# Exidekat/TransformerUpscaler

Hardware: AMD Instinct MI355X
Metric: images/sec, FastTransformer 2x 720p->1080p inference (higher is better)
Workload: dtype bf16

## Files before the change

include/tupscale_hip.h:

```cpp
#ifndef TUPSCALE_HIP_H
#define TUPSCALE_HIP_H

#ifdef __cplusplus
extern "C" {
#endif

int tup_abi_version(void);

int tup_conv3x3_c3_fwd(const float* x, const void* wp, const float* bias, const float* in_mask,
                       const void* out_mask, void* out, int B, int H, int W, int relu, void* stream);

int tup_conv3x3_c64_fwd(const void* x, const void* wp, const float* bias, const void* add,
                        const void* mask, void* out, int B, int H, int W, int ntiles, int r,
                        int cout_valid, int relu, int out_mode, int in_r, void* stream);

int tup_conv5x5_c64_planar_fwd(const void* x, const void* wp, const float* bias, const void* wv,
                               const float* bv, float* out, int B, int H, int W, int r, int relu, void* stream);

int tup_conv3x3_planar_fwd(const float* x, const float* w28, const float* bias, const float* add,
                           float* out, int B, int H, int W, int r, int clamp01, void* stream);

int tup_resize_aa_fwd(const float* in, float* out, const int* ymin, const int* ysize, const float* yw,
                      int KY, const int* xmin, const int* xsize, const float* xw, int KX, int planes,
                      int Hi, int Wi, int Ho, int Wo, int clamp01, void* stream);

int tup_tail_stream_r2_fwd(const float* x, const float* wfu_t, const float* bfu, const float* wfc_t, const float* bfc,
                           const float* ui, float* out, int B, int H, int W, int clamp01, void* stream);

int tup_tail_stream_r2_resize_fwd(const float* x, const float* wfu_t, const float* bfu, const float* wfc_t, const float* bfc,
                                  const float* ui, float* out, const int* ymin, const int* ysize, const float* yw, int KY,
                                  const int* xmin, const int* xsize, const float* xw, int KX, const int* oxb, const int* oyb,
                                  int B, int H, int W, int Ho, int Wo, int sc, int band_h, int ext, int clamp01, void* stream);

int tup_tail_fused_fwd(const float* x, const float* wfu, const float* bfu, const float* wfc, const float* bfc,
                       const float* ui, float* out, const int* ymin, const int* ysize, const float* yw, int KY,
                       const int* xmin, const int* xsize, const float* xw, int KX, int B, int H, int W, int r,
                       int Ho, int Wo, int EH, int EW, int clamp01, void* stream);

int tup_clamp01_fwd(const float* in, float* out, long long n, void* stream);

int tup_layernorm_fwd(const float* x, const float* gamma, const float* beta, void* y,
                      float* mean, float* rstd, int M, void* stream);

int tup_relpos_bias_expand(const float* table, float* frag, void* stream);

int tup_window_attn_fwd(const void* qkv, const float* bias_frag, void* out, float* lse, int nwin, float drop_p,
                        unsigned int drop_seed, void* stream);

int tup_gemm_tokens_fwd(const void* A, int a_dtype, int lda, const void* Wt, const float* bias,
                        const float* res, const void* aux, void* out, int ldo, int M, int N, int K,
                        int epilogue, float drop_p, unsigned int drop_seed, void* stream);

int tup_ln_gemm_fwd(const float* x, const float* gamma, const float* beta, const void* Wt,
                    const float* bias, void* out, int M, int N, void* stream);

int tup_fused_mlp_fwd(float* x, const float* gamma, const float* beta, const void* w1, const float* b1,
                      const void* w2, const float* b2, int M, void* stream);

int tup_patch_embed_fwd(const void* feat, const void* Wt, const float* bias, float* x_out,
                        int B, int H, int W, void* stream);

int tup_patch_unembed_fwd(const void* x, int x_bf16, const void* Wt, const float* bias, const void* skip,
                          void* out, int B, int H, int W, void* stream);


int tup_rt_patch_embed_fwd(const void* feat, const void* Wt, const float* bias, const float* pos, float* x_out,
                           int B, int H, int W, void* stream);
// ... 154 lines not shown
```

transformerupscaler_amd/_lib.py:

```python
from __future__ import annotations

import ctypes
import os
from ctypes import c_float, c_int, c_longlong, c_uint, c_void_p

_HERE = os.path.dirname(os.path.abspath(__file__))
LIB_PATH = os.environ.get("TUP_LIB_PATH") or os.path.join(_HERE, "libtupscale_hip.so")
ABI_VERSION = 15

P = c_void_p
I = c_int
F = c_float
U = c_uint

SIGNATURES = {
    "tup_abi_version": [],
    "tup_conv3x3_c3_fwd": [P, P, P, P, P, P, I, I, I, I, P],
    "tup_conv3x3_c64_fwd": [P, P, P, P, P, P, I, I, I, I, I, I, I, I, I, P],
    "tup_conv5x5_c64_planar_fwd": [P, P, P, P, P, P, I, I, I, I, I, P],
    "tup_conv3x3_planar_fwd": [P, P, P, P, P, I, I, I, I, I, P],
    "tup_resize_aa_fwd": [P, P, P, P, P, I, P, P, P, I, I, I, I, I, I, I, P],
    "tup_tail_fused_fwd": [P, P, P, P, P, P, P, P, P, P, I, P, P, P, I, I, I, I, I, I, I, I, I, I, P],
    "tup_tail_stream_r2_fwd": [P, P, P, P, P, P, P, I, I, I, I, P],
    "tup_tail_stream_r2_resize_fwd": [P] * 7 + [P, P, P, I, P, P, P, I, P, P] + [I] * 9 + [P],
    "tup_clamp01_fwd": [P, P, c_longlong, P],
    "tup_layernorm_fwd": [P, P, P, P, P, P, I, P],
    "tup_relpos_bias_expand": [P, P, P],
    "tup_window_attn_fwd": [P, P, P, P, I, F, U, P],
    "tup_gemm_tokens_fwd": [P, I, I, P, P, P, P, P, I, I, I, I, I, F, U, P],
    "tup_ln_gemm_fwd": [P, P, P, P, P, P, I, I, P],
    "tup_fused_mlp_fwd": [P, P, P, P, P, P, P, I, P],
    "tup_patch_embed_fwd": [P, P, P, P, I, I, I, P],
    "tup_patch_unembed_fwd": [P, I, P, P, P, P, I, I, I, P],
    "tup_rt_patch_embed_fwd": [P, P, P, P, P, I, I, I, P],
    "tup_rt_patch_unembed_fwd": [P, P, P, P, P, I, I, I, P],
    "tup_rt_attention_fwd": [P, P, P, I, I, F, U, P],
    "tup_rt_attention_bwd": [P, P, P, P, P, P, I, I, F, U, P],
    "tup_layernorm128_fwd": [P, P, P, P, P, P, I, P],
    "tup_layernorm128_bwd": [P, P, P, P, P, P, P, P, P, I, P, F, U, P],
    "tup_rt_patch_wgrad": [P, P, P, I, I, I, P],
    "tup_conv3x3_c64_wgrad_s2d": [P, P, P, P, I, I, I, I, I, P],
    "tup_rt_bicubic_bwd": [P] * 10 + [I, I, I, I, I, P],
    "tup_rt_bicubic_bwd_banded": [P] * 7 + [I, P, P, I, P, P, I, I, I, I, I, P, P],
    "tup_relpos_bias_expand_h": [P, P, I, P],
    "tup_relpos_bias_expand_n_h": [P, P, I, P],
    "tup_window_attn_bwd_h": [P, P, P, P, P, P, P, P, I, I, F, U, P],
    "tup_relpos_bias_reduce_h": [P, P, I, P],
    "tup_wt_patch_wgrad": [P, P, P, I, I, I, I, P],
    "tup_window_attn_fwd_h": [P, P, P, P, I, I, F, U, P],
    "tup_wt_patch_embed_fwd": [P, P, P, P, I, I, I, I, P],
    "tup_wt_patch_unembed_fwd": [P, P, P, P, P, I, I, I, I, P],
    "tup_fused_qkv_attn_fwd": [P, P, P, P, P, P, P, I, P],
    "tup_fused_attn_block_fwd": [P, P, P, P, P, P, P, P, I, P],
    "tup_fused_block_fwd": [P] * 10 + [I, P],
    "tup_fused_blocks32_fwd": [P, P, I, I, P],
    "tup_blocks_stream_fwd": [P, P, P, I, I, P],
    "tup_clock_probe": [P, P],
    "tup_pack_gather": [P, P, I, P, P, c_longlong, I, P],
    "tup_adam_step": [P, P, I, P],
    "tup_l1_loss_partial": [P, P, P, c_longlong, I, P],
    "tup_l1_loss_bwd": [P, P, P, P, c_longlong, P],
    "tup_u8hwc_to_f32chw": [P, P, I, I, I, I, P],
    "tup_f32chw_to_u8hwc": [P, P, I, I, I, I, P],
    "tup_bra_compose": [P, P, P, P, P, P, P, P],
    "tup_bra_backward": [P, P, P, P, P, P, P, P, P, I, I, I, P],
    "tup_bra_chain": [P, P, P, P, P, P, P, P, P, P, P],
    "tup_resize_u8_rows": [P, P, P, P, P, I, I, I, I, I, P],
    "tup_resize_u8_cols": [P, P, P, P, P, P, I, I, I, I, I, I, P],
    "tup_rt_bicubic_sum_fwd": [P, P, P, P, P, P, P, P, P, P, P, I, I, I, I, I, I, I, I, P],
    "tup_quality_f32_partial": [P, P, P, I, I, I, I, F, P],
    "tup_quality_u8hwc_partial": [P, P, P, I, I, I, I, F, P],
    "tup_quality_reduce": [P, P, I, I, I, I, F, P],
# ... 69 lines not shown
```

transformerupscaler_amd/csrc/check_resources.py:

```python
#!/usr/bin/env python3
import json
import os
import re
import subprocess
import sys

GUARDED = [
    ("fused_attn.hip", ["fused_qkv_attn_kernel"]),
    ("block_stream.hip", ["blocks_stream_kernel"]),
    ("fused_blocks.hip", ["fused_mlp_v2_kernel"]),
    ("conv3x3_c64.hip", ["conv_c64_persistent_kernel", "bra_rows_persistent_kernel", "conv3_thin_rows_kernel"]),
    ("conv_thin.hip", ["conv3x3_c3_persistent_kernel"]),
    ("gemm_tokens.hip", ["gemm_panel2_kernel", "patch_embed_kernel"]),
    ("conv_bwd.hip", ["conv3x3_wgrad_c64_kernel", "conv3x3_wgrad_thin_kernel"]),
    ("branch_a_train.hip", ["bra_wgrad_kernel"]),
    ("gemm_wgrad.hip", ["gemm_wgrad_wide_kernel"]),
]
EXEMPT = re.compile(r"fused_qkv_attn_kernel<true, true, true>|fused_qkv_attn_kernelILb1ELb1ELb1E|fused_mlp_v2_kernelILi[1-9]|blocks_stream_kernel<true>|blocks_stream_kernelILb1E")
ALLOWED_BYTES = {"fused_mlp_v2_kernelILi0E": 72}

FIELDS = {
    "sgprs": r"TotalSGPRs: (\d+)", "vgprs": r" VGPRs: (\d+)", "agprs": r"AGPRs: (\d+)",
    "scratch_bytes_per_lane": r"ScratchSize \[bytes/lane\]: (\d+)", "waves_per_simd": r"Occupancy \[waves/SIMD\]: (\d+)",
    "sgpr_spill": r"SGPRs Spill: (\d+)", "vgpr_spill": r"VGPRs Spill: (\d+)",
}


def demangle(names):
    try:
        out = subprocess.run(["c++filt"], input="\n".join(names), capture_output=True, text=True, check=True).stdout.split("\n")
        return dict(zip(names, out))
    except Exception:
        return {n: n for n in names}


def parse(path):
    txt = open(path, errors="replace").read()
    parts = re.split(r"remark: Function Name: (\S+)", txt)
    recs = {}
    for name, body in zip(parts[1::2], parts[2::2]):
        rec = {}
        for k, pat in FIELDS.items():
            m = re.search(pat, body)
            if m:
                rec[k] = int(m.group(1))
        recs[name] = rec
    return recs


def main(argv):
    out_path = None
    files = []
    for a in argv:
        if a.startswith("--out="):
            out_path = a[6:]
        else:
            files.append(a)
    report, bad = {}, []
    for f in sorted(files):
        src = os.path.basename(f).replace(".remarks", ".hip")
        recs = parse(f)
        names = demangle(list(recs))
        for mangled, rec in recs.items():
            nice = names.get(mangled, mangled)
            rec["source"] = src
# ... 32 lines not shown
```

transformerupscaler_amd/engine.py:

```python
from __future__ import annotations

import os

import math
from typing import Dict, Optional, Tuple

import torch

from . import ops
from .weights import BLOCKS, VALID_SCALES, upsampler_layout


stage_timer = None
fuse_attention = 3


class _NullCtx:
    def __enter__(self):
        return None

    def __exit__(self, *a):
        return False


def _stage(name: str):
    return stage_timer(name) if stage_timer is not None else _NullCtx()


def resolve_scale(h: int, w: int, res_out, upscale_factor: Optional[int]):
    if upscale_factor is not None:
        res_out = (h * upscale_factor, w * upscale_factor)
    else:
        upscale_factor = math.ceil(max(res_out[0] / h, res_out[1] / w))
    if upscale_factor not in VALID_SCALES:
        raise ValueError(f"Requested scale={upscale_factor} was not built.")
    return (int(res_out[0]), int(res_out[1])), int(upscale_factor)


blocks_in_one_launch = True
stream_blocks = True
STREAM_MIN_WINDOWS = 512
stream_bf16_tokens = True
fuse_blocks = True
fuse_tail = True
stream_tail = True


def _block_operands(pk, i, bias_frags):
    return (pk[f"b{i}.qkv.whn"], pk[f"b{i}.qkv.bhn"], bias_frags[i], pk[f"b{i}.proj.wpp"], pk[f"b{i}.proj.b"],
            pk[f"b{i}.fc1.wfqn"], pk[f"b{i}.fc1.bqn"], pk[f"b{i}.fc2.wh4"], pk[f"b{i}.fc2.b"])


def transformer_blocks(pk: Dict[str, torch.Tensor], x: torch.Tensor, bias_frags, capture=None, bf16_out: bool = False):
    if (fuse_blocks and fuse_attention >= 3 and capture is None and "b0.stream.0" in pk and blocks_in_one_launch and stream_blocks
            and x.shape[0] // 64 >= STREAM_MIN_WINDOWS):
        table = ops.stream_table([tuple(pk[f"b{i}.stream.{j}"] for j in range(7)) for i in range(BLOCKS)])
        return ops.blocks_stream(x, table, out_bf16=bf16_out and stream_bf16_tokens)
    if fuse_blocks and fuse_attention >= 3 and capture is None and "b0.proj.wpp" in pk and blocks_in_one_launch:
        table = ops.block_table([_block_operands(pk, i, bias_frags) for i in range(BLOCKS)])
        return ops.fused_blocks32(x, table)
    for i in range(BLOCKS):
        qkv = None
        if fuse_blocks and fuse_attention >= 3 and capture is None and f"b{i}.proj.wpp" in pk:
            ops.fused_block(x, *_block_operands(pk, i, bias_frags))
            continue
        if fuse_blocks and fuse_attention == 2 and capture is None and f"b{i}.proj.wpp" in pk:
            ops.fused_attn_block(x, pk[f"b{i}.norm1.w"], pk[f"b{i}.norm1.b"], pk[f"b{i}.qkv.wh"], pk[f"b{i}.qkv.bh"], bias_frags[i],
                                 pk[f"b{i}.proj.wpp"], pk[f"b{i}.proj.b"])
            ops.fused_mlp(x, pk[f"b{i}.norm2.w"], pk[f"b{i}.norm2.b"], pk[f"b{i}.fc1.wfq"], pk[f"b{i}.fc1.bq"],
                          pk[f"b{i}.fc2.wh4"], pk[f"b{i}.fc2.b"])
            continue
        if fuse_blocks and fuse_attention and capture is None and f"b{i}.qkv.wh" in pk:
            att = ops.fused_qkv_attn(x, pk[f"b{i}.norm1.w"], pk[f"b{i}.norm1.b"], pk[f"b{i}.qkv.wh"], pk[f"b{i}.qkv.bh"], bias_frags[i])
        else:
            if fuse_blocks:
                qkv = ops.ln_gemm(x, pk[f"b{i}.norm1.w"], pk[f"b{i}.norm1.b"], pk[f"b{i}.qkv.w"], pk[f"b{i}.qkv.b"])
            else:
                y = ops.layernorm(x, pk[f"b{i}.norm1.w"], pk[f"b{i}.norm1.b"])
                qkv = ops.gemm_tokens(y, pk[f"b{i}.qkv.w"], pk[f"b{i}.qkv.b"], "bf16")
            att = ops.window_attn(qkv, bias_frags[i])
        ops.gemm_tokens(att, pk[f"b{i}.proj.w"], pk[f"b{i}.proj.b"], "res", res=x, out=x)
        if fuse_blocks and f"b{i}.fc1.wfq" in pk:
            ops.fused_mlp(x, pk[f"b{i}.norm2.w"], pk[f"b{i}.norm2.b"], pk[f"b{i}.fc1.wfq"], pk[f"b{i}.fc1.bq"],
                          pk[f"b{i}.fc2.wh4"], pk[f"b{i}.fc2.b"])
        else:
            y = ops.layernorm(x, pk[f"b{i}.norm2.w"], pk[f"b{i}.norm2.b"])
            hid = ops.gemm_tokens(y, pk[f"b{i}.fc1.w"], pk[f"b{i}.fc1.b"], "gelu")
            ops.gemm_tokens(hid, pk[f"b{i}.fc2.w"], pk[f"b{i}.fc2.b"], "res", res=x, out=x)
        if capture is not None:
            capture[f"block{i}"] = x.clone()
            capture[f"block{i}_qkv"] = qkv
            capture[f"block{i}_attn_out"] = att
    return x


def forward(pk: Dict[str, torch.Tensor], bias_frags, x: torch.Tensor, scale: int, res_out: Tuple[int, int],
            require_ratio: bool = True, capture: Optional[dict] = None, fuse_branch_a: bool = True) -> torch.Tensor:
    cap = capture
    x = x.contiguous().float()
    B, _, H, W = x.shape
    with _stage("conv1"):
        feat1 = ops.conv1(x, pk["conv1.w"], pk["conv1.b"], relu=True)
    with _stage("conv2"):
        feat = ops.conv_c64(feat1, pk["conv2.w"], pk["conv2.b"], 1, relu=True)
    del feat1
    stages = upsampler_layout(scale)
    up = feat
    if fuse_branch_a and "bra.w" in pk:
        for si, (_, r) in enumerate(stages[:-1]):
            up = ops.conv_c64(up, pk[f"up1.{si}.w"], pk[f"up1.{si}.b"], r, relu=False)
        with _stage("branch_a"):
            upscaled_input = ops.branch_a_composed(up, pk["bra.w"], pk["bra.b"], pk["bra.wv"], pk["bra.bv"], stages[-1][1])
    else:
        for si, (_, r) in enumerate(stages):
            with _stage(f"up1.{si}"):
                up = ops.conv_c64(up, pk[f"up1.{si}.w"], pk[f"up1.{si}.b"], r, relu=False)
        upscaled_input = ops.conv_c64_thin(up, pk["up1_conv.w"], None, 3, relu=True)
        if cap is not None:
            cap["up1"] = up
    if cap is not None:
        cap["feat"] = feat; cap["upscaled_input"] = upscaled_input
    del up
    with _stage("patch_embed"):
        xw = ops.patch_embed(feat, pk["pe.w"], pk["pe.b"])
    if cap is not None:
        cap["win_in"] = xw.clone()
    with _stage("blocks"):
        xw = transformer_blocks(pk, xw, bias_frags, cap, bf16_out=cap is None)
    with _stage("unembed"):
        combined = ops.patch_unembed(xw, pk["pu.w"], pk["pu.b"], feat)
    with _stage("dec1"):
        dec = ops.conv_c64(combined, pk["dec1.w"], pk["dec1.b"], 1, relu=True)
    with _stage("dec2"):
        residual = ops.conv_c64_thin(dec, pk["dec2.w"], pk["dec2.b"], 3, relu=False)
    if cap is not None:
        cap["combined"] = combined; cap["dec"] = dec; cap["residual"] = residual
    t = residual
    hs, ws = H * scale, W * scale
    needs_resize = bool(require_ratio) and tuple(res_out) != (hs, hs) and tuple(res_out) != (hs, ws)
    fu = upsampler_layout(scale)
    if fuse_tail and cap is None:
        for si, (_, r) in enumerate(fu[:-1]):
            t = ops.conv_planar(t, pk[f"fu.{si}.w"], pk[f"fu.{si}.b"], r)
        li = len(fu) - 1
        if (stream_tail and fu[li][1] == 2 and "tail.wfu_t" in pk
                and ops.tail_stream_fits(t.shape[0], t.shape[2], t.shape[3], tuple(res_out) if needs_resize else None)):
            with _stage("tail"):
                out = ops.tail_stream_r2(t, pk["tail.wfu_t"], pk[f"fu.{li}.b"], pk["tail.wfc_t"], pk["fuc.b"], upscaled_input,
                                         clamp=True, out_hw=tuple(res_out) if needs_resize else None)
                if out is None:
                    out = ops.tail_stream_r2(t, pk["tail.wfu_t"], pk[f"fu.{li}.b"], pk["tail.wfc_t"], pk["fuc.b"], upscaled_input, clamp=False)
                    out = ops.resize_aa(out, tuple(res_out), clamp=True)
            return out
        with _stage("tail"):
            out = ops.tail_fused(t, pk[f"fu.{li}.w"], pk[f"fu.{li}.b"], pk["fuc.w"], pk["fuc.b"], upscaled_input, fu[li][1],
                                 tuple(res_out) if needs_resize else (hs, ws), clamp=True)
        return out
    for si, (_, r) in enumerate(fu):
        t = ops.conv_planar(t, pk[f"fu.{si}.w"], pk[f"fu.{si}.b"], r)
    out = ops.conv_planar(t, pk["fuc.w"], pk["fuc.b"], 1, add=upscaled_input, clamp=not needs_resize)
    if cap is not None:
        cap["sum"] = out
    if needs_resize:
        out = ops.resize_aa(out, res_out, clamp=True)
    return out
```

transformerupscaler_amd/ops.py:

```python
from __future__ import annotations

import os

import numpy as np
import torch

from . import _lib
from .resize_taps import aa_taps

BF16, F32 = torch.bfloat16, torch.float32


_raw_stream = getattr(torch._C, "_cuda_getCurrentRawStream", None)
_cur_dev = torch.cuda.current_device


def _stream():
    if _raw_stream is not None:
        return _raw_stream(_cur_dev())
    return torch.cuda.current_stream().cuda_stream


def _chk(t: torch.Tensor, dtype, shape=None, name="tensor"):
    if t.dtype != dtype:
# ... 25 lines not shown


def zero_pool_end():
    global _zero_pool
    _zero_pool = None


def _zeros(shape, device):
    n = 1
    for d in shape:
        n *= int(d)
    zp = _zero_pool
    if zp is not None and zp[0].device == torch.device(device) and zp[1] + n <= zp[0].numel():
        off = zp[1]
        zp[1] = off + ((n + 63) // 64) * 64
        return zp[0][off:off + n].view(shape)
    return torch.zeros(shape, dtype=F32, device=device)


def conv1(x, wp, bias, relu=True, in_mask=None, out_mask=None):
    B, C, H, W = x.shape
    assert C == 3
    out = torch.empty((B, H, W, 64), dtype=BF16, device=x.device)
    _lib.call("tup_conv3x3_c3_fwd", _chk(x, F32, None, "x"), _chk(wp, BF16, (64, 32), "wp"),
              _opt(bias, F32, (64,), "bias"), _opt(in_mask, F32, x.shape, "in_mask"),
              _opt(out_mask, BF16, out.shape, "out_mask"), out.data_ptr(), B, H, W, int(relu), _stream())
    return out


def conv_c64(x, wp, bias, r=1, relu=False, add=None, mask=None, in_r=1, out=None):
    B, Hi, Wi, C = x.shape
    assert C == 64 and Hi % in_r == 0 and Wi % in_r == 0
    H, W = Hi // in_r, Wi // in_r
    nt = r * r
    if out is None:
        out = torch.empty((B, H * r, W * r, 64), dtype=BF16, device=x.device)
    else:
        _chk(out, BF16, (B, H * r, W * r, 64), "out")
    _lib.call("tup_conv3x3_c64_fwd", _chk(x, BF16, None, "x"), _chk(wp, BF16, (nt, in_r * in_r, 9, 64, 64), "wp"),
              _opt(bias, F32, (nt, 64), "bias"), _opt(add, BF16, out.shape, "add"), _opt(mask, BF16, out.shape, "mask"),
              out.data_ptr(), B, H, W, nt, r, 64, int(relu), 0, in_r, _stream())
    return out


def conv_c64_thin(x, wp, bias, cout, relu=False, out=None):
    B, H, W, C = x.shape
    assert C == 64 and 1 <= cout <= 16
    if out is None:
        out = torch.empty((B, cout, H, W), dtype=F32, device=x.device)
    else:
        _chk(out, F32, (B, cout, H, W), "out")
    _lib.call("tup_conv3x3_c64_fwd", _chk(x, BF16, None, "x"), _chk(wp, BF16, (1, 1, 9, 16, 64), "wp"),
              _opt(bias, F32, (cout,), "bias"), None, None, out.data_ptr(), B, H, W, 1, 1, cout, int(relu), 1, 1, _stream())
    return out


def branch_a_composed(x, wp, bias, wv, bv, r, relu=True):
    B, H, W, C = x.shape
    assert C == 64 and r in (2, 3, 6)
    rows, n = {2: 16, 3: 32, 6: 112}[r], 3 * r * r
    out = torch.empty((B, 3, H * r, W * r), dtype=F32, device=x.device)
    _lib.call("tup_conv5x5_c64_planar_fwd", _chk(x, BF16, None, "x"), _chk(wp, BF16, (1, 1, 25, rows, 64), "wp"),
              _chk(bias, F32, (n,), "bias"), _chk(wv, BF16, (9, n, 25, 64), "wv"), _chk(bv, F32, (9, n), "bv"),
              out.data_ptr(), B, H, W, r, int(relu), _stream())
    return out


def conv_planar(x, w28, bias, r=1, add=None, clamp=False):
    B, C, H, W = x.shape
    assert C == 3
    cout = 3 * r * r
    both = clamp == "both"
    shape = (B, 3, H * r, W * r)
    out = torch.empty(((2,) if both else ()) + shape, dtype=F32, device=x.device)
    _lib.call("tup_conv3x3_planar_fwd", _chk(x, F32, None, "x"), _chk(w28, F32, (cout, 28), "w28"),
              _opt(bias, F32, (cout,), "bias"), _opt(add, F32, shape, "add"), out.data_ptr(),
              B, H, W, r, 2 if both else int(bool(clamp)), _stream())
    return (out[0], out[1]) if both else out


_TAP_CACHE = {}


def _taps_on(device, in_size, out_size):
    key = (str(device), in_size, out_size)
    if key not in _TAP_CACHE:
        lo, n, w, k = aa_taps(in_size, out_size)
        _TAP_CACHE[key] = (torch.from_numpy(lo).to(device), torch.from_numpy(n).to(device),
                           torch.from_numpy(w).to(device), k)
    return _TAP_CACHE[key]


def resize_aa(x, size, clamp=False):
    B, C, Hi, Wi = x.shape
    Ho, Wo = size
    ylo, yn, yw, ky = _taps_on(x.device, Hi, Ho)
    xlo, xn, xw, kx = _taps_on(x.device, Wi, Wo)
    both = clamp == "both"
    out = torch.empty(((2,) if both else ()) + (B, C, Ho, Wo), dtype=F32, device=x.device)
    _lib.call("tup_resize_aa_fwd", _chk(x, F32, None, "x"), out.data_ptr(), ylo.data_ptr(), yn.data_ptr(),
              yw.data_ptr(), ky, xlo.data_ptr(), xn.data_ptr(), xw.data_ptr(), kx, B * C, Hi, Wi, Ho, Wo,
              2 if both else int(bool(clamp)), _stream())
    return (out[0], out[1]) if both else out


TAIL_TILE_H = 16
# ... 900 lines not shown
```

transformerupscaler_amd/packing.py:

```python
from __future__ import annotations

from typing import Dict

import torch

from .weights import BLOCKS, upsampler_layout

_PERM64 = torch.tensor([((n >> 2) & 3) * 16 + (n >> 4) * 4 + (n & 3) for n in range(64)], dtype=torch.long)


_IDX_CACHE: Dict[tuple, torch.Tensor] = {}


def _dev_index(key, build, device) -> torch.Tensor:
    k = (key, str(device))
    t = _IDX_CACHE.get(k)
    if t is None:
        t = _IDX_CACHE[k] = build().to(device)
    return t


def _perm64(device) -> torch.Tensor:
    return _dev_index("perm64", lambda: _PERM64, device)


def perm_rows64(w: torch.Tensor) -> torch.Tensor:
    n = w.shape[0]
    assert n % 64 == 0
    idx = _dev_index(("rows64", n), lambda: (torch.arange(n // 64).view(-1, 1) * 64 + _PERM64.view(1, -1)).reshape(-1), w.device)
    return w.index_select(0, idx)


def pack_conv_c64(weight: torch.Tensor, bias, r: int):
    cout, cin = weight.shape[0], weight.shape[1]
    assert cin == 64 and cout == 64 * r * r and weight.shape[2:] == (3, 3)
    w = weight.reshape(64, r * r, 64, 9)
    w = w.permute(1, 3, 0, 2)
    w = w.index_select(2, _perm64(w.device))
    b = None if bias is None else bias.reshape(64, r * r).t().contiguous().float()
    return w.unsqueeze(1).contiguous().to(torch.bfloat16), b


def pack_conv_c64_thin(weight: torch.Tensor):
    co = weight.shape[0]
    assert weight.shape[1] == 64 and co <= 16
    w = torch.zeros(9, 16, 64, dtype=weight.dtype, device=weight.device)
    w[:, :co, :] = weight.reshape(co, 64, 9).permute(2, 0, 1)
    return w.view(1, 1, 9, 16, 64).contiguous().to(torch.bfloat16)


def pack_conv1(weight: torch.Tensor):
    assert tuple(weight.shape) == (64, 3, 3, 3)
    w = torch.zeros(64, 32, dtype=weight.dtype, device=weight.device)
    w[:, :27] = weight.permute(0, 2, 3, 1).reshape(64, 27)
    return perm_rows64(w).contiguous().to(torch.bfloat16)


def pack_planar(weight: torch.Tensor):
    cout = weight.shape[0]
    assert weight.shape[1:] == (3, 3, 3)
    w = torch.zeros(cout, 28, dtype=torch.float32, device=weight.device)
    w[:, :27] = weight.reshape(cout, 27).float()
    return w.contiguous()


def pack_planar_t(weight: torch.Tensor):
    cout = weight.shape[0]
    assert weight.shape[1:] == (3, 3, 3)
    w = torch.zeros(27, (cout + 3) // 4 * 4, dtype=torch.float32, device=weight.device)
    w[:, :cout] = weight.reshape(cout, 27).float().t()
    return w.contiguous()


def pack_linear(weight: torch.Tensor):
    return perm_rows64(weight).contiguous().to(torch.bfloat16)


def pack_linear_stack(weights, transpose: bool = False):
    w = torch.stack([t.detach() for t in weights])
    if transpose:
        w = w.transpose(1, 2)
    n = w.shape[1]
    assert n % 64 == 0
    idx = _dev_index(("rows64", n), lambda: (torch.arange(n // 64).view(-1, 1) * 64 + _PERM64.view(1, -1)).reshape(-1), w.device)
    return w.index_select(1, idx).to(torch.bfloat16)


def pack_fc1_fused(weight: torch.Tensor):
    return pack_linear(weight).index_select(1, _fused_k_order(weight.device)).contiguous()


def pack_fc1_fused_q(weight: torch.Tensor, bias: torch.Tensor):
    return pack_fc1_fused(weight.detach() * 0.25), (bias.detach().float() * 0.25).contiguous()


def pack_fc2_h4(weight: torch.Tensor):
    return perm_rows64(weight.detach() * 4.0).contiguous().to(torch.float16)


def fold_layernorm(weight: torch.Tensor, bias: torch.Tensor, gamma: torch.Tensor, beta: torch.Tensor):
    w = weight.detach().float()
# ... 199 lines not shown
        k = f"up1.upsamplers.{scale}.{idx}"
        pk[f"up1.{si}.w"], pk[f"up1.{si}.b"] = pack_conv_c64(sd[k + ".weight"].detach(), sd[k + ".bias"].detach(), r)
        k = f"final_upscale.upsamplers.{scale}.{idx}"
        pk[f"fu.{si}.w"] = pack_planar(sd[k + ".weight"].detach()); pk[f"fu.{si}.b"] = f32(sd[k + ".bias"])
    pk["up1_conv.w"] = pack_conv_c64_thin(sd["up1_conv.conv.weight"].detach())
    if not backward:
        idx, r = upsampler_layout(scale)[-1]
        k = f"up1.upsamplers.{scale}.{idx}"
        pk["bra.w"], pk["bra.b"], pk["bra.wv"], pk["bra.bv"] = pack_branch_a(
            sd[k + ".weight"].detach(), sd[k + ".bias"].detach(), sd["up1_conv.conv.weight"].detach(), r)
    pk["fuc.w"] = pack_planar(sd["final_upscale_conv.weight"].detach()); pk["fuc.b"] = f32(sd["final_upscale_conv.bias"])
    if not backward and upsampler_layout(scale)[-1][1] == 2:
        li = len(upsampler_layout(scale)) - 1
        pk["tail.wfu_t"] = pack_planar_t(sd[f"final_upscale.upsamplers.{scale}.{upsampler_layout(scale)[-1][0]}.weight"].detach())
        pk["tail.wfc_t"] = pack_planar_t(sd["final_upscale_conv.weight"].detach())
    pk["pe.w"] = pack_patch_embed(sd["patch_embed.weight"].detach()); pk["pe.b"] = f32(sd["patch_embed.bias"])
    for i in range(BLOCKS):
        p = f"window_blocks.{i}"
        for nm in ("norm1", "norm2"):
            pk[f"b{i}.{nm}.w"] = f32(sd[f"{p}.{nm}.weight"]); pk[f"b{i}.{nm}.b"] = f32(sd[f"{p}.{nm}.bias"])
        pk[f"b{i}.table"] = f32(sd[f"{p}.attn.relative_position_bias_table"])
        for nm, key in (("qkv", "attn.qkv"), ("proj", "attn.proj"), ("fc1", "mlp.0"), ("fc2", "mlp.2")):
            pk[f"b{i}.{nm}.b"] = f32(sd[f"{p}.{key}.bias"])
    for nm, key in (("qkv", "attn.qkv"), ("proj", "attn.proj"), ("fc1", "mlp.0"), ("fc2", "mlp.2")):
        ws = [sd[f"window_blocks.{i}.{key}.weight"] for i in range(BLOCKS)]
        wp = pack_linear_stack(ws)
        for i in range(BLOCKS):
            pk[f"b{i}.{nm}.w"] = wp[i]
        if backward:
            wt = pack_linear_stack(ws, transpose=True)
            for i in range(BLOCKS):
                pk[f"b{i}.{nm}.wd"] = wt[i]
    if not backward:
        for i in range(BLOCKS):
            p = f"window_blocks.{i}"
            pk[f"b{i}.qkv.wh"], pk[f"b{i}.qkv.bh"] = pack_qkv_heads(sd[f"{p}.attn.qkv.weight"], sd[f"{p}.attn.qkv.bias"])
            pk[f"b{i}.proj.wpp"] = pack_proj_pairs(sd[f"{p}.attn.proj.weight"])
            pk[f"b{i}.fc1.wfq"], pk[f"b{i}.fc1.bq"] = pack_fc1_fused_q(sd[f"{p}.mlp.0.weight"], sd[f"{p}.mlp.0.bias"])
            pk[f"b{i}.qkv.whn"], pk[f"b{i}.qkv.bhn"] = pack_qkv_heads(*fold_layernorm(
                sd[f"{p}.attn.qkv.weight"], sd[f"{p}.attn.qkv.bias"], sd[f"{p}.norm1.weight"], sd[f"{p}.norm1.bias"]))
            pk[f"b{i}.fc1.wfqn"], pk[f"b{i}.fc1.bqn"] = pack_fc1_fused_q(*fold_layernorm(
                sd[f"{p}.mlp.0.weight"], sd[f"{p}.mlp.0.bias"], sd[f"{p}.norm2.weight"], sd[f"{p}.norm2.bias"]))
            pk[f"b{i}.fc2.wh4"] = pack_fc2_h4(sd[f"window_blocks.{i}.mlp.2.weight"])
            for j, t in enumerate(pack_stream_block(
                    sd[f"{p}.attn.qkv.weight"], sd[f"{p}.attn.qkv.bias"], sd[f"{p}.norm1.weight"], sd[f"{p}.norm1.bias"],
                    sd[f"{p}.attn.relative_position_bias_table"], sd[f"{p}.attn.proj.weight"], sd[f"{p}.attn.proj.bias"],
                    sd[f"{p}.mlp.0.weight"], sd[f"{p}.mlp.0.bias"], sd[f"{p}.norm2.weight"], sd[f"{p}.norm2.bias"],
                    sd[f"{p}.mlp.2.weight"], sd[f"{p}.mlp.2.bias"])):
                pk[f"b{i}.stream.{j}"] = t
    pk["pu.w"] = pack_patch_unembed(sd["patch_unembed.weight"].detach()); pk["pu.b"] = f32(sd["patch_unembed.bias"])
    pk["dec1.w"], pk["dec1.b"] = pack_conv_c64(sd["decoder_conv1.weight"].detach(), sd["decoder_conv1.bias"].detach(), 1)
    pk["dec2.w"] = pack_conv_c64_thin(sd["decoder_conv2.weight"].detach()); pk["dec2.b"] = f32(sd["decoder_conv2.bias"])
    if not backward:
        return pk
    t = lambda k: sd[k].detach()
    pk["conv1.wd"] = pack_conv_c64_thin(t("conv1.weight").flip(2, 3).transpose(0, 1).contiguous())
    pk["conv2.wd"] = pack_conv_c64_dgrad(t("conv2.weight"), 1)
    pk["dec1.wd"] = pack_conv_c64_dgrad(t("decoder_conv1.weight"), 1)
    pk["dec2.wd"] = pack_conv_thin_dgrad(t("decoder_conv2.weight"))
    pk["up1_conv.wd"] = pack_conv_thin_dgrad(t("up1_conv.conv.weight"))
    pk["fuc.wd"] = pack_planar_dgrad(t("final_upscale_conv.weight"))
    for si, (idx, r) in enumerate(upsampler_layout(scale)):
        pk[f"up1.{si}.wd"] = pack_conv_c64_dgrad(t(f"up1.upsamplers.{scale}.{idx}.weight"), r)
        pk[f"fu.{si}.raw"] = f32(sd[f"final_upscale.upsamplers.{scale}.{idx}.weight"])
    pk["pe.wd"] = pack_linear(t("patch_embed.weight").permute(2, 3, 1, 0).reshape(4096, 192))
    pk["pu.wd"] = pack_linear(t("patch_unembed.weight").permute(0, 2, 3, 1).reshape(192, 4096))
    return pk


def pack_conv_c64_stride2(weight: torch.Tensor, bias):
    assert tuple(weight.shape) == (64, 64, 3, 3)
    w = torch.zeros(4, 9, 64, 64, dtype=weight.dtype, device=weight.device)
    for si in range(2):
        for sj in range(2):
            for dy in range(3):
                for dx in range(3):
                    ky, kx = 2 * (dy - 1) + si + 1, 2 * (dx - 1) + sj + 1
                    if 0 <= ky <= 2 and 0 <= kx <= 2:
                        w[si * 2 + sj, dy * 3 + dx] = weight[:, :, ky, kx]
    w = w.index_select(2, _perm64(w.device))
    b = None if bias is None else bias.reshape(1, 64).contiguous().float()
    return w.unsqueeze(0).contiguous().to(torch.bfloat16), b


def pack_conv_c64_stride2_dgrad(weight: torch.Tensor):
    assert tuple(weight.shape) == (64, 64, 3, 3)
    w = torch.zeros(4, 9, 64, 64, dtype=weight.dtype, device=weight.device)
    for si in range(2):
        for sj in range(2):
            for dy in range(3):
                for dx in range(3):
                    ky, kx = si + 1 - 2 * (dy - 1), sj + 1 - 2 * (dx - 1)
                    if 0 <= ky <= 2 and 0 <= kx <= 2:
                        w[si * 2 + sj, dy * 3 + dx] = weight[:, :, ky, kx].t()
    w = w.index_select(2, _perm64(w.device))
    return w.unsqueeze(1).contiguous().to(torch.bfloat16)


def unpack_conv_c64_stride2_wgrad(dwp: torch.Tensor):
    dw = torch.zeros(64, 64, 3, 3, dtype=dwp.dtype, device=dwp.device)
    for si in range(2):
        for sj in range(2):
            for dy in range(3):
                for dx in range(3):
                    ky, kx = 2 * (dy - 1) + si + 1, 2 * (dx - 1) + sj + 1
                    if 0 <= ky <= 2 and 0 <= kx <= 2:
# ... 78 lines not shown
```

Measured before the change: 2353.

## Fuse decoder conv1 and conv2 into one persistent kernel with seam fixup

```diff
diff --git a/include/tupscale_hip.h b/include/tupscale_hip.h
--- a/include/tupscale_hip.h
+++ b/include/tupscale_hip.h
@@ -13,6 +13,9 @@
 int tup_conv3x3_c64_fwd(const void* x, const void* wp, const float* bias, const void* add,
                         const void* mask, void* out, int B, int H, int W, int ntiles, int r,
                         int cout_valid, int relu, int out_mode, int in_r, void* stream);
+
+int tup_decoder_fused_fwd(const void* x, const void* w1, const float* b1, const void* wz, const float* b2,
+                          float* seamv, float* cseam, float* out, int B, int H, int W, void* stream);
 
 int tup_conv5x5_c64_planar_fwd(const void* x, const void* wp, const float* bias, const void* wv,
                                const float* bv, float* out, int B, int H, int W, int r, int relu, void* stream);
diff --git a/transformerupscaler_amd/_lib.py b/transformerupscaler_amd/_lib.py
--- a/transformerupscaler_amd/_lib.py
+++ b/transformerupscaler_amd/_lib.py
@@ -18,6 +18,7 @@
     "tup_conv3x3_c3_fwd": [P, P, P, P, P, P, I, I, I, I, P],
     "tup_conv3x3_c64_fwd": [P, P, P, P, P, P, I, I, I, I, I, I, I, I, I, P],
     "tup_conv5x5_c64_planar_fwd": [P, P, P, P, P, P, I, I, I, I, I, P],
+    "tup_decoder_fused_fwd": [P, P, P, P, P, P, P, P, I, I, I, P],
     "tup_conv3x3_planar_fwd": [P, P, P, P, P, I, I, I, I, I, P],
     "tup_resize_aa_fwd": [P, P, P, P, P, I, P, P, P, I, I, I, I, I, I, I, P],
     "tup_tail_fused_fwd": [P, P, P, P, P, P, P, P, P, P, I, P, P, P, I, I, I, I, I, I, I, I, I, I, P],
diff --git a/transformerupscaler_amd/csrc/check_resources.py b/transformerupscaler_amd/csrc/check_resources.py
--- a/transformerupscaler_amd/csrc/check_resources.py
+++ b/transformerupscaler_amd/csrc/check_resources.py
@@ -11,6 +11,7 @@
     ("fused_blocks.hip", ["fused_mlp_v2_kernel"]),
     ("conv3x3_c64.hip", ["conv_c64_persistent_kernel", "bra_rows_persistent_kernel", "conv3_thin_rows_kernel"]),
     ("conv_thin.hip", ["conv3x3_c3_persistent_kernel"]),
+    ("decoder_fused.hip", ["decoder_fused_kernel"]),
     ("gemm_tokens.hip", ["gemm_panel2_kernel", "patch_embed_kernel"]),
     ("conv_bwd.hip", ["conv3x3_wgrad_c64_kernel", "conv3x3_wgrad_thin_kernel"]),
     ("branch_a_train.hip", ["bra_wgrad_kernel"]),
diff --git a/transformerupscaler_amd/csrc/decoder_fused.hip b/transformerupscaler_amd/csrc/decoder_fused.hip
--- /dev/null
+++ b/transformerupscaler_amd/csrc/decoder_fused.hip
@@ -0,0 +1,343 @@
+#include "common.h"
+
+namespace {
+
+constexpr int TH = 8, TW = 32, HALO_W = TW + 2, HALO_H = TH + 2, NPIX_HALO = HALO_H * HALO_W;
+constexpr int IN_BYTES = NPIX_HALO * 128, IN_CHUNKS = NPIX_HALO * 8;
+constexpr int WROWS = 64, WSLAB = WROWS * 128, WCHUNKS = 9 * WROWS * 8;
+constexpr size_t DEC_LDS = (size_t)9 * WSLAB + 2 * (size_t)IN_BYTES + 256;
+static_assert(DEC_LDS <= 163840, "LDS budget");
+
+__device__ __attribute__((aligned(16))) unsigned int dec_zero_line[4] = {0u, 0u, 0u, 0u};
+
+#define TUP_ADD_DPP(a, v, ctrl) asm("v_add_f32_dpp %0, %1, %0 " ctrl " row_mask:0xf bank_mask:0xf bound_ctrl:1" : "+v"(a) : "v"(v))
+
+__global__ __launch_bounds__(512, 2) void decoder_fused_kernel(
+    const bf16_t* __restrict__ x, const bf16_t* __restrict__ wp, const float* __restrict__ bias,
+    const bf16_t* __restrict__ wz, float* __restrict__ part, float* __restrict__ seamv, float* __restrict__ cseam,
+    int B, int H, int W, int tilesX, int tilesY)
+{
+    extern __shared__ __attribute__((aligned(16))) char smem[];
+    char* w_lds = smem;
+    char* in_lds = smem + 9 * WSLAB;
+
+    const int grp = __builtin_amdgcn_readfirstlane((int)(threadIdx.x >> 8));
+    const int tid = threadIdx.x & 255, lane = tid & 63, wave = tid >> 6;
+    const int g = lane >> 4, p = lane & 15;
+    const int total_tiles = tilesX * tilesY * B;
+    char* my_in = in_lds + grp * IN_BYTES;
+
+    constexpr int NPIECE = (IN_CHUNKS + 255) / 256;
+    int rel[NPIECE];
+#pragma unroll
+    for (int it = 0; it < NPIECE; ++it) {
+        const int idx = min(it * 256 + tid, IN_CHUNKS - 1);
+        const int q = idx >> 3, c = (idx & 7) ^ ((q >> 1) & 7);
+        const int yy = q / HALO_W, xx = q - yy * HALO_W;
+        rel[it] = ((yy - 1) * W + (xx - 1)) * 128 + c * 16;
+    }
+    const bool last_ok = (NPIECE - 1) * 256 + tid < IN_CHUNKS;
+    struct TC { int tx, ty, b; };
+    auto prefetch_tile = [&](const TC& c) {
+        const int ty0 = c.ty * TH, tx0 = c.tx * TW;
+        const char* xb = reinterpret_cast<const char*>(x + (size_t)c.b * H * W * 64);
+        if (ty0 >= 1 && ty0 + TH + 1 <= H && tx0 >= 1 && tx0 + TW + 1 <= W) {
+            const char* tb = xb + ((size_t)ty0 * W + tx0) * 128;
+#pragma unroll
+            for (int it = 0; it < NPIECE; ++it) {
+                if (it == NPIECE - 1 && !last_ok) continue;
+                __builtin_amdgcn_global_load_lds((const __attribute__((address_space(1))) void*)(tb + rel[it]),
+                                                 (__attribute__((address_space(3))) void*)(my_in + (it * 256 + wave * 64) * 16), 16, 0, 0);
+            }
+            return;
+        }
+#pragma unroll 1
+        for (int base = 0; base < IN_CHUNKS; base += 256) {
+            const int idx = base + tid;
+            if (idx < IN_CHUNKS) {
+                const int q = idx >> 3, cphys = idx & 7;
+                const int c = cphys ^ ((q >> 1) & 7);
+                const int yy = q / HALO_W, xx = q - yy * HALO_W;
+                const int iy = ty0 - 1 + yy, ix = tx0 - 1 + xx;
+                const void* src = (iy >= 0 && iy < H && ix >= 0 && ix < W)
+                                      ? (const void*)(xb + ((size_t)(iy * W + ix) * 128 + c * 16)) : (const void*)dec_zero_line;
+                __builtin_amdgcn_global_load_lds((const __attribute__((address_space(1))) void*)src,
+                                                 (__attribute__((address_space(3))) void*)(my_in + (base + wave * 64) * 16), 16, 0, 0);
+            }
+        }
+    };
+
+    uint32_t poff[9][2];
+#pragma unroll
+    for (int tap = 0; tap < 9; ++tap)
+#pragma unroll
+        for (int rw = 0; rw < 2; ++rw)
+            poff[tap][rw] = lds_addr(my_in) + (uint32_t)swz128((2 * wave + rw) * HALO_W + p + (tap / 3) * HALO_W + (tap % 3), g);
+    const uint32_t wbase0 = lds_addr(w_lds) + (uint32_t)swz128(p, g), wbase1 = wbase0 ^ 64u;
+    const uint32_t wbase0h = wbase0 + 57344u, wbase1h = wbase1 + 57344u;
+
+    f32x4 acc[4][4];
+    float* bias_lds = reinterpret_cast<float*>(in_lds + 2 * IN_BYTES);
+    const uint32_t bias_addr = lds_addr(bias_lds) + (uint32_t)(g * 64);
+    bf16x8 zf[3][2];
+    const uint32_t wz_voff = (uint32_t)(p * 128 + g * 16);
+    auto load_zf = [&]() {
+#pragma unroll
+        for (int dy = 0; dy < 3; ++dy) {
+            const bf16_t* base = wz + dy * 1024;
+            asm volatile("global_load_dwordx4 %0, %1, %2" : "=v"(zf[dy][0]) : "v"(wz_voff), "s"(base));
+            asm volatile("global_load_dwordx4 %0, %1, %2 offset:64" : "=v"(zf[dy][1]) : "v"(wz_voff), "s"(base));
+        }
+    };
+
+    auto compute_tile = [&]() {
+#pragma unroll
+        for (int ct = 0; ct < 4; ++ct) acc[0][ct] = __builtin_bit_cast(f32x4, lds_read_b128_asm(bias_addr + ct * 16));
+        lds_wait<0>();
+#pragma unroll
+        for (int pg = 1; pg < 4; ++pg)
+#pragma unroll
+            for (int ct = 0; ct < 4; ++ct) acc[pg][ct] = acc[0][ct];
+        constexpr int NSTEPS = 18, PER = 8;
+        bf16x8 pf[3][4], wf[3][4];
+        auto load_one = [&](int step, int slot, int j) {
+            const int tap = step >> 1;
+            if (j < 4) {
+                pf[slot][j] = (step & 1) ? lds_read_b128_asm_off_x64(poff[tap][j >> 1], (j & 1) * 2048)
+                                         : lds_read_b128_asm_off(poff[tap][j >> 1], (j & 1) * 2048);
+            } else {
+                const int woff = (tap * WROWS + (j - 4) * 16) * 128;
+                wf[slot][j - 4] = woff < 57344 ? lds_read_b128_asm_off((step & 1) ? wbase1 : wbase0, woff)
+                                               : lds_read_b128_asm_off((step & 1) ? wbase1h : wbase0h, woff - 57344);
+            }
+        };
+#pragma unroll
+        for (int j = 0; j < PER; ++j) load_one(0, 0, j);
+#pragma unroll
+        for (int j = 0; j < PER; ++j) load_one(1, 1, j);
+#pragma unroll
+        for (int step = 0; step < NSTEPS; ++step) {
+            const int cur = step % 3;
+            if (step + 1 < NSTEPS) lds_wait<PER>(); else lds_wait<0>();
+            __builtin_amdgcn_sched_barrier(0);
+            int rd = 0;
+#pragma unroll
+            for (int m = 0; m < 16; ++m) {
+                if (step + 2 < NSTEPS) {
+#pragma unroll
+                    for (int j = 0; j < PER; ++j)
+                        if (j == rd && j * 16 <= m * PER) { load_one(step + 2, (step + 2) % 3, j); ++rd; }
+                }
+                const int pg = m / 4, ct = m % 4;
+                acc[pg][ct] = mfma16x16x32(wf[cur][ct], pf[cur][pg], acc[pg][ct]);
+                __builtin_amdgcn_sched_barrier(0);
+            }
+        }
+    };
+
+    auto store_tile = [&](const TC& c) {
+        const int b = c.b, y0 = c.ty * TH + 2 * wave, x0 = c.tx * TW;
+        const bool edge = c.ty * TH + TH > H || x0 + TW > W;
+        f32x4 z[4][3];
+#pragma unroll
+        for (int pg = 0; pg < 4; ++pg) {
+            typedef short s16x2 __attribute__((ext_vector_type(2)));
+            uint32_t pk[8];
+#pragma unroll
+            for (int ct = 0; ct < 4; ++ct) {
+                pk[ct * 2 + 0] = pack_bf16x2(acc[pg][ct][0], acc[pg][ct][1]);
+                pk[ct * 2 + 1] = pack_bf16x2(acc[pg][ct][2], acc[pg][ct][3]);
+            }
+#pragma unroll
+            for (int q = 0; q < 8; ++q)
+                pk[q] = __builtin_bit_cast(uint32_t, __builtin_elementwise_max(__builtin_bit_cast(s16x2, pk[q]), s16x2{0, 0}));
+            if (edge) {
+                const bool ok = y0 + (pg >> 1) < H && x0 + (pg & 1) * 16 + p < W;
+#pragma unroll
+                for (int q = 0; q < 8; ++q) pk[q] = ok ? pk[q] : 0u;
+            }
+            const bf16x8 b0 = __builtin_bit_cast(bf16x8, u32x4{pk[0], pk[1], pk[2], pk[3]});
+            const bf16x8 b1 = __builtin_bit_cast(bf16x8, u32x4{pk[4], pk[5], pk[6], pk[7]});
+#pragma unroll
+            for (int dy = 0; dy < 3; ++dy) {
+                z[pg][dy] = mfma16x16x32(zf[dy][0], b0, f32x4{0.f, 0.f, 0.f, 0.f});
+                z[pg][dy] = mfma16x16x32(zf[dy][1], b1, z[pg][dy]);
+            }
+        }
+        __builtin_amdgcn_sched_barrier(0);
+        asm volatile("s_nop 7\n\ts_nop 7\n\ts_nop 4" ::: "memory");
+        __builtin_amdgcn_sched_barrier(0);
+        float h[2][2][3];
+#pragma unroll
+        for (int rw = 0; rw < 2; ++rw)
+#pragma unroll
+            for (int dy = 0; dy < 3; ++dy) {
+                const f32x4 l = z[2 * rw][dy], r = z[2 * rw + 1][dy];
+                float v0 = l[1], v1 = r[1];
+                TUP_ADD_DPP(v0, l[0], "row_shr:1"); TUP_ADD_DPP(v0, l[2], "row_shl:1"); TUP_ADD_DPP(v0, r[2], "row_shr:15");
+                TUP_ADD_DPP(v1, r[0], "row_shr:1"); TUP_ADD_DPP(v1, r[2], "row_shl:1"); TUP_ADD_DPP(v1, l[0], "row_shl:15");
+                h[rw][0][dy] = v0; h[rw][1][dy] = v1;
+            }
+        const bool live = g < 3;
+        const int plane = H * W, nrec = 3 * plane * 4;
+        const __amdgpu_buffer_rsrc_t rp = __builtin_amdgcn_make_buffer_rsrc(part + (size_t)b * 3 * plane, 0, nrec, 0x00020000);
+        const __amdgpu_buffer_rsrc_t rs = __builtin_amdgcn_make_buffer_rsrc(seamv + (size_t)b * 3 * plane, 0, nrec, 0x00020000);
+        const int crec = H * tilesX * 128;
+        const __amdgpu_buffer_rsrc_t rc = __builtin_amdgcn_make_buffer_rsrc(cseam + (size_t)b * H * tilesX * 32, 0, crec, 0x00020000);
+        const int cbase = (g * plane + y0 * W) * 4;
+#pragma unroll
+        for (int cg = 0; cg < 2; ++cg) {
+            const int ox = x0 + cg * 16 + p;
+            const bool colok = live && ox < W;
+            const int o = cbase + ox * 4, rowb = W * 4;
+            const float o0 = h[0][cg][1] + h[1][cg][2], o1 = h[0][cg][0] + h[1][cg][1];
+            __builtin_amdgcn_raw_buffer_store_b32(__builtin_bit_cast(uint32_t, o0), rp, colok && y0 < H ? o : nrec, 0, 0);
+            __builtin_amdgcn_raw_buffer_store_b32(__builtin_bit_cast(uint32_t, o1), rp, colok && y0 + 1 < H ? o + rowb : nrec, 0, 0);
+            __builtin_amdgcn_raw_buffer_store_b32(__builtin_bit_cast(uint32_t, h[0][cg][2]), rs,
+                                                  colok && y0 >= 1 && y0 < H ? o - rowb : nrec, 0, 0);
+            __builtin_amdgcn_raw_buffer_store_b32(__builtin_bit_cast(uint32_t, h[1][cg][0]), rs,
+                                                  colok && y0 + 2 < H ? o + 2 * rowb : nrec, 0, 0);
+        }
+#pragma unroll
+        for (int rw = 0; rw < 2; ++rw) {
+            const int y = y0 + rw;
+            const bool left = p == 0;
+            const f32x4 v = left ? f32x4{z[2 * rw][0][2], z[2 * rw][1][2], z[2 * rw][2][2], 0.f}
+                                 : f32x4{z[2 * rw + 1][0][0], z[2 * rw + 1][1][0], z[2 * rw + 1][2][0], 0.f};
+            const bool ok = live & (y < H) & (left | ((p == 15) & (x0 + TW <= W)));
+            const int off = ((y * tilesX + c.tx) * 2 + (left ? 0 : 1)) * 64 + g * 16;
+            __builtin_amdgcn_raw_buffer_store_b128(__builtin_bit_cast(u32x4, v), rc, ok ? off : crec, 0, 0);
+        }
+    };
+    constexpr int NSTORES = 10;
+
+    int first, first0, stride, limit;
+    if ((gridDim.x & 7) == 0) {
+        const int per = gridDim.x >> 3, band = (total_tiles + 7) >> 3, start = (blockIdx.x & 7) * band;
+        limit = min(total_tiles, start + band);
+        first0 = start + (blockIdx.x >> 3);
+        first = first0 + grp * per;
+        stride = 2 * per;
+    } else {
+        limit = total_tiles;
+        first0 = blockIdx.x;
+        first = first0 + grp * gridDim.x;
+        stride = 2 * gridDim.x;
+    }
+    const int my_count = first < limit ? (limit - first + stride - 1) / stride : 0;
+    const int cnt0 = first0 < limit ? (limit - first0 + stride - 1) / stride : 0;
+    const int nphases = 2 * cnt0 + 1;
+    TC c_first;
+    { const int t = first / tilesX; c_first.tx = first - t * tilesX; c_first.ty = t % tilesY; c_first.b = t / tilesY; }
+    const int step_x = stride % tilesX, step_y = (stride / tilesX) % tilesY, step_b = stride / (tilesX * tilesY);
+    auto advance = [&](TC& c) {
+        c.tx += step_x;
+        if (c.tx >= tilesX) { c.tx -= tilesX; ++c.ty; }
+        c.ty += step_y; c.b += step_b;
+        if (c.ty >= tilesY) { c.ty -= tilesY; ++c.b; }
+    };
+
+    for (int idx = threadIdx.x; idx < WCHUNKS; idx += 512) {
+        const int row = idx >> 3, c = idx & 7;
+        *reinterpret_cast<u32x4*>(w_lds + swz128(row, c)) = *reinterpret_cast<const u32x4*>(wp + (size_t)idx * 8);
+    }
+    if (threadIdx.x < 64) {
+        const int gg = threadIdx.x >> 4, ct = (threadIdx.x >> 2) & 3, e = threadIdx.x & 3;
+        bias_lds[threadIdx.x] = bias[gg * 16 + ct * 4 + e];
+    }
+    if (grp == 0 && my_count > 0) prefetch_tile(c_first);
+    __syncthreads();
+    TC c_done = c_first, c_next = c_first;
+    if (grp == 0) advance(c_next);
+
+    for (int ph = 0; ph < nphases; ++ph) {
+        const int k = ph >> 1;
+        if ((ph & 1) == grp) {
+            if (k < my_count) compute_tile();
+        } else {
+            const int done = grp == 0 ? k : k - 1;
+            const int nxt = done + 1;
+            const bool store = done >= 0 && done < my_count;
+            const bool fetch = nxt < my_count;
+            if (store) load_zf();
+            if (fetch) prefetch_tile(c_next);
+            if (store) {
+                if (fetch) asm volatile("s_waitcnt vmcnt(%0)" ::"n"(NPIECE - 1) : "memory");
+                else asm volatile("s_waitcnt vmcnt(0)" ::: "memory");
+                store_tile(c_done);
+                asm volatile("s_waitcnt vmcnt(%0)" ::"n"(NSTORES) : "memory");
+            } else {
+                asm volatile("s_waitcnt vmcnt(0)" ::: "memory");
+            }
+            c_done = c_next;
+            advance(c_next);
+        }
+        asm volatile("s_waitcnt lgkmcnt(0)" ::: "memory");
+        __builtin_amdgcn_s_barrier();
+    }
+    asm volatile("s_waitcnt vmcnt(0)" ::: "memory");
+}
+
+template <int V>
+__global__ __launch_bounds__(256) void decoder_finish_kernel(
+    float* __restrict__ res, const float* __restrict__ seamv, const float* __restrict__ cseam, const float* __restrict__ bias,
+    int H, int W, int tilesX)
+{
+    typedef float fv __attribute__((ext_vector_type(V)));
+    const int x0 = (blockIdx.x * 256 + threadIdx.x) * V;
+    if (x0 >= W) return;
+    const int row = blockIdx.y, b = row / H, y = row - b * H;
+    const size_t plane = (size_t)H * W;
+    const int ys = (y & 1) ? y + 1 : y - 1;
+    const bool has_seam = ys >= 0 && ys < H;
+    const size_t o0 = (size_t)b * 3 * plane + (size_t)y * W + x0;
+#pragma unroll
+    for (int c = 0; c < 3; ++c) {
+        const size_t o = o0 + c * plane;
+        fv v = *reinterpret_cast<const fv*>(res + o);
+        const fv sv = has_seam ? *reinterpret_cast<const fv*>(seamv + o) : fv{};
+#pragma unroll
+        for (int e = 0; e < V; ++e) {
+            const int xq = x0 + e;
+            float t = bias[c] + v[e];
+            if (has_seam) t += sv[e];
+            int ctile = -1, side = 0;
+            if ((xq & 31) == 31 && xq + 1 < W) { ctile = (xq >> 5) + 1; side = 0; }
+            else if ((xq & 31) == 0 && xq > 0) { ctile = (xq >> 5) - 1; side = 1; }
+            if (ctile >= 0) {
+#pragma unroll
+                for (int dy = 0; dy < 3; ++dy) {
+                    const int yy = y + dy - 1;
+                    if (yy >= 0 && yy < H) t += cseam[((((size_t)b * H + yy) * tilesX + ctile) * 2 + side) * 16 + c * 4 + dy];
+                }
+            }
+            v[e] = t;
+        }
+        *reinterpret_cast<fv*>(res + o) = v;
+    }
+}
+
+}
+
+extern "C" int tup_decoder_fused_fwd(const void* x, const void* w1, const float* b1, const void* wz, const float* b2,
+                                     float* seamv, float* cseam, float* out, int B, int H, int W, void* stream)
+{
+    if (B <= 0 || H <= 0 || W <= 0) return 0;
+    const int tilesX = (W + TW - 1) / TW, tilesY = (H + TH - 1) / TH;
+    const long long nt = (long long)tilesX * tilesY * B;
+    if (nt > 0x7fffffffLL || (long long)H * W * 12 > 0x7fffffffLL || (long long)H * tilesX * 128 > 0x7fffffffLL)
+        return (int)hipErrorInvalidValue;
+    hipStream_t s = reinterpret_cast<hipStream_t>(stream);
+    TUP_SET_DYN_LDS(decoder_fused_kernel, DEC_LDS);
+    const int grid = (int)(nt < 256 ? nt : 256);
+    decoder_fused_kernel<<<dim3(grid), dim3(512), DEC_LDS, s>>>((const bf16_t*)x, (const bf16_t*)w1, b1, (const bf16_t*)wz, out,
+                                                                 seamv, cseam, B, H, W, tilesX, tilesY);
+    TUP_CHECK_LAUNCH();
+    if ((long long)B * H > 0x7fffffffLL) return (int)hipErrorInvalidValue;
+    if (W % 4 == 0)
+        decoder_finish_kernel<4><<<dim3((unsigned)((W / 4 + 255) / 256), (unsigned)(B * H)), dim3(256), 0, s>>>(out, seamv, cseam, b2, H, W, tilesX);
+    else
+        decoder_finish_kernel<1><<<dim3((unsigned)((W + 255) / 256), (unsigned)(B * H)), dim3(256), 0, s>>>(out, seamv, cseam, b2, H, W, tilesX);
+    TUP_CHECK_LAUNCH();
+    return 0;
+}
diff --git a/transformerupscaler_amd/engine.py b/transformerupscaler_amd/engine.py
--- a/transformerupscaler_amd/engine.py
+++ b/transformerupscaler_amd/engine.py
@@ -44,6 +44,7 @@
 fuse_blocks = True
 fuse_tail = True
 stream_tail = True
+fuse_decoder = True
 
 
 def _block_operands(pk, i, bias_frags):
@@ -129,10 +130,14 @@
         xw = transformer_blocks(pk, xw, bias_frags, cap, bf16_out=cap is None)
     with _stage("unembed"):
         combined = ops.patch_unembed(xw, pk["pu.w"], pk["pu.b"], feat)
-    with _stage("dec1"):
-        dec = ops.conv_c64(combined, pk["dec1.w"], pk["dec1.b"], 1, relu=True)
-    with _stage("dec2"):
-        residual = ops.conv_c64_thin(dec, pk["dec2.w"], pk["dec2.b"], 3, relu=False)
+    if fuse_decoder and fuse_tail and cap is None and "dec2.wz" in pk:
+        with _stage("decoder"):
+            residual = ops.decoder_fused(combined, pk["dec1.w"], pk["dec1.b"], pk["dec2.wz"], pk["dec2.b"])
+    else:
+        with _stage("dec1"):
+            dec = ops.conv_c64(combined, pk["dec1.w"], pk["dec1.b"], 1, relu=True)
+        with _stage("dec2"):
+            residual = ops.conv_c64_thin(dec, pk["dec2.w"], pk["dec2.b"], 3, relu=False)
     if cap is not None:
         cap["combined"] = combined; cap["dec"] = dec; cap["residual"] = residual
     t = residual
diff --git a/transformerupscaler_amd/ops.py b/transformerupscaler_amd/ops.py
--- a/transformerupscaler_amd/ops.py
+++ b/transformerupscaler_amd/ops.py
@@ -101,6 +101,18 @@
         _chk(out, F32, (B, cout, H, W), "out")
     _lib.call("tup_conv3x3_c64_fwd", _chk(x, BF16, None, "x"), _chk(wp, BF16, (1, 1, 9, 16, 64), "wp"),
               _opt(bias, F32, (cout,), "bias"), None, None, out.data_ptr(), B, H, W, 1, 1, cout, int(relu), 1, 1, _stream())
+    return out
+
+
+def decoder_fused(x, w1, b1, wz, b2):
+    B, H, W, C = x.shape
+    assert C == 64
+    out = torch.empty((B, 3, H, W), dtype=F32, device=x.device)
+    seamv = torch.empty((B, 3, H, W), dtype=F32, device=x.device)
+    cseam = torch.empty((B, H, (W + 31) // 32, 32), dtype=F32, device=x.device)
+    _lib.call("tup_decoder_fused_fwd", _chk(x, BF16, None, "x"), _chk(w1, BF16, (1, 1, 9, 64, 64), "w1"), _chk(b1, F32, (1, 64), "b1"),
+              _chk(wz, BF16, (48, 64), "wz"), _chk(b2, F32, (3,), "b2"), seamv.data_ptr(), cseam.data_ptr(), out.data_ptr(),
+              B, H, W, _stream())
     return out
 
 
diff --git a/transformerupscaler_amd/packing.py b/transformerupscaler_amd/packing.py
--- a/transformerupscaler_amd/packing.py
+++ b/transformerupscaler_amd/packing.py
@@ -47,6 +47,15 @@
     w = torch.zeros(9, 16, 64, dtype=weight.dtype, device=weight.device)
     w[:, :co, :] = weight.reshape(co, 64, 9).permute(2, 0, 1)
     return w.view(1, 1, 9, 16, 64).contiguous().to(torch.bfloat16)
+
+
+def pack_dec2_scatter(weight: torch.Tensor):
+    assert tuple(weight.shape) == (3, 64, 3, 3)
+    kk = torch.arange(64)
+    ch = 16 * ((kk % 32) // 8) + 8 * (kk // 32) + kk % 8
+    w = torch.zeros(3, 4, 4, 64, dtype=weight.dtype, device=weight.device)
+    w[:, :3, :3, :] = weight[:, ch.to(weight.device), :, :].permute(2, 0, 3, 1)
+    return w.reshape(48, 64).contiguous().to(torch.bfloat16)
 
 
 def pack_conv1(weight: torch.Tensor):
@@ -352,6 +361,7 @@
     pk["dec1.w"], pk["dec1.b"] = pack_conv_c64(sd["decoder_conv1.weight"].detach(), sd["decoder_conv1.bias"].detach(), 1)
     pk["dec2.w"] = pack_conv_c64_thin(sd["decoder_conv2.weight"].detach()); pk["dec2.b"] = f32(sd["decoder_conv2.bias"])
     if not backward:
+        pk["dec2.wz"] = pack_dec2_scatter(sd["decoder_conv2.weight"].detach())
         return pk
     t = lambda k: sd[k].detach()
     pk["conv1.wd"] = pack_conv_c64_thin(t("conv1.weight").flip(2, 3).transpose(0, 1).contiguous())
```

After: 2477 (median of 6 runs). 5.2% higher.
